# ypear/crdt

Measured on AMD Instinct MI355X. Metric: CRDT items merged/sec at 1/2/4/8 MI355X + % of HBM roofline, higher is better.
Workload: dtype u8/u32 (integer byte-stream + index work)

## Files before the change

crdt_amd/csrc/yc_decode.hip:

```cpp
#include <algorithm>
#include <cstdlib>

#include "yc_work.h"

namespace yc {

__device__ __forceinline__ uint64_t win8(const uint8_t* __restrict__ b, uint32_t p) {
  const uint32_t* d = (const uint32_t*)(b + (p & ~3u));
  return ((uint64_t)d[0] | ((uint64_t)d[1] << 32)) >> ((p & 3u) * 8);
}
__device__ __forceinline__ uint32_t win4(const uint8_t* __restrict__ b, uint32_t p) {
  const uint32_t* d = (const uint32_t*)(b + (p & ~3u));
  return __builtin_amdgcn_alignbyte(d[1], d[0], p & 3u);
}
struct RegWin {
  uint32_t r0, r1, r2, r3, r4, r5;
  uint32_t T;
  __device__ __forceinline__ static uint32_t sel(uint32_t m, uint32_t a1, uint32_t a0) { return (a1 & m) | (a0 & ~m); }
  __device__ __forceinline__ uint32_t word(uint32_t k) const {
    const uint32_t m0 = 0u - (k & 1u), m1 = 0u - ((k >> 1) & 1u), m2 = 0u - ((k >> 2) & 1u);
    const uint32_t a0 = sel(m0, r1, r0), a1 = sel(m0, r3, r2), a2 = sel(m0, r5, r4);
    return sel(m2, a2, sel(m1, a1, a0));
  }
  __device__ __forceinline__ uint32_t byte(uint32_t i) const { return (word(i >> 2) >> ((i & 3u) * 8)) & 0xFFu; }
// ... 3025 lines not shown
  const int pr = parse_struct<true, 32, WinSrc, DEFER>(WinSrc{bw, slot, s0}, p, uend, 0xFFFFFFFFu, &v);
  if (DEFER && pr == PARSE_DEFER) {
    w.sd_defer[atomicAdd(&w.ctr->nsd_defer, 1u)] = i;
    return;
  }
  if (pr <= 0) { raise_err(err, pr == -1 ? ERR_UNSUPPORTED : ERR_DECODE); return; }
  const uint32_t ref0 = v.ref;
  if (sec.pad && !w.lazy) {
    v.info = (uint8_t)((v.info & 0xE0u) | REF_SKIP);
    v.ref = REF_SKIP;
  }
  w.s_len[i] = v.len;
  w.s_info[i] = v.info;
  w.s_cidx[i] = sec.cidx;
  uint32_t oc = NONE, rc = NONE;
  const bool item = v.ref != REF_GC && v.ref != REF_SKIP;
  if (item && (v.info & 0x80u)) {
    oc = w.lazy ? v.oc : v.oc == sec.client ? sec.cidx : find_client(w, nclients, doc, v.oc);
    if (oc == NONE && !w.lazy) oc = UNKNOWN;
  }
  if (item && (v.info & 0x40u)) {
    rc = w.lazy ? v.rc : v.rc == sec.client ? sec.cidx : find_client(w, nclients, doc, v.rc);
    if (rc == NONE && !w.lazy) rc = UNKNOWN;
  }
  w.s_ocidx[i] = oc;
  w.s_oclock[i] = v.ok_;
  w.s_rcidx[i] = rc;
  if (rc != NONE) w.s_rclock[i] = v.rk;
  uint32_t pk = item ? v.pkind : 0u, pa = NONE, pb = 0;
  if (pk == 1) { pa = v.pa; pb = v.pb; }
  else if (pk == 2) {
    pa = w.lazy ? v.pa : v.pa == sec.client ? sec.cidx : find_client(w, nclients, doc, v.pa);
    pb = v.pb;
    if (pa == NONE && !w.lazy) pa = UNKNOWN;
  }
  if (pk != 0 && !v.has_psub) w.ctr->narray_roots = 1;
  if (pk == 2) w.ctr->nested = 1;
  wave_flag(&w.ctr->any_rorigin, item && (v.info & 0x40u));
  wave_count_add_sharded(w.ctr->nroots_sh, pk != 0);
  bool canon_hdr = true;
  if (item) {
    uint32_t h = 0;
    if (v.info & 0x80u) h += vu_size(v.oc) + vu_size(v.ok_);
    if (v.info & 0x40u) h += vu_size(v.rc) + vu_size(v.rk);
    if ((v.info & 0xC0u) == 0) {
      h += 1;
      if (v.pkind == 1) h += vu_size(v.pn) + v.pn;
      else h += vu_size(v.pa) + vu_size(v.pb);
      if (v.has_psub) h += vu_size(v.psn) + v.psn;
    }
    canon_hdr = h == v.cpos - p0 - 1;
  }
  w.s_pk[i] = (uint8_t)(pk | (canon_hdr ? 0u : 0x80u) | ((v.anyf & ANY_REENCODE) ? 0x40u : 0u) | ((v.anyf & ANY_KEYS) ? 0x20u : 0u));
  if (pk != 0) {
    w.s_pa[i] = pa;
    w.s_pb[i] = pb;
    w.s_psub[i] = v.has_psub ? v.psub_pos : NONE;
    w.s_psublen[i] = v.psub_len;
  }
  w.s_cpos[i] = v.cpos;
  w.s_cend[i] = v.cend;
  uint32_t celem = v.cpos;
  if (v.ref == REF_ANY || v.ref == REF_JSON) celem += vu_size(v.nel);
  w.s_celem[i] = celem;
  wave_flag(&w.ctr->any_json, ref0 == REF_JSON || ref0 == REF_EMBED || ref0 == REF_FORMAT || (v.anyf & ANY_KEYS) != 0);
}
__global__ __launch_bounds__(256) __attribute__((amdgpu_waves_per_eu(8, 8))) void k_struct_decode(Work w, uint32_t nstructs) {
  __shared__ __attribute__((aligned(16))) uint32_t win[256 * SD_STRIDE];
  const uint32_t i = blockIdx.x * blockDim.x + threadIdx.x;
  if (i < nstructs) struct_decode_one<true>(w, i, win);
}
constexpr uint32_t SD_DEFER_GRID = 1024;
__global__ __launch_bounds__(256) void k_struct_decode_deferred(Work w) {
  __shared__ __attribute__((aligned(16))) uint32_t win[256 * SD_STRIDE];
  const uint32_t n = w.ctr->nsd_defer;
  for (uint32_t k = blockIdx.x * blockDim.x + threadIdx.x; k < n; k += gridDim.x * blockDim.x)
    struct_decode_one<false>(w, w.sd_defer[k], win);
}
__global__ __launch_bounds__(256) void k_json_structs(Work w, uint32_t nstructs) {
  const uint32_t i = blockIdx.x * blockDim.x + threadIdx.x;
  if (i >= nstructs) return;
  const uint8_t* __restrict__ bw = struct_bytes(w, i);
  const uint32_t ref = bw[w.s_pos[i]] & 31u;
  if (w.ntrusted && w.sections[w.s_sec[i]].upd < w.ntrusted) return;
  if (ref == REF_ANY && (w.s_pk[i] & 0x20u)) {
    if (w.jskip_any) return;
    if (!any_keys_exact(bw, w.s_cpos[i], w.s_cend[i])) return;
    const uint32_t k = atomicAdd(&w.ctr->njson, 1u);
    if (k < w.jcap) w.jlist[k] = i;
    return;
  }
  if (ref != REF_JSON && ref != REF_EMBED && ref != REF_FORMAT) return;
  const int jr = json_content(bw, w.s_cpos[i], w.s_cend[i], ref);
  if (jr > 0) raise_err(&w.ctr->err, ERR_DECODE);
  if (jr < 0) {
    const uint32_t k = atomicAdd(&w.ctr->njson, 1u);
    if (k < w.jcap) w.jlist[k] = i;
  }
}
void launch_json_structs(const Work& w, uint32_t nstructs, hipStream_t s) {
  if (nstructs) hipLaunchKernelGGL(k_json_structs, dim3(nstructs / 256 + 1), dim3(256), 0, s, w, nstructs);
}
__global__ __launch_bounds__(64) void k_json_canon(Work w, const uint32_t* __restrict__ list, uint32_t n, JItem* __restrict__ items,
                                                   uint32_t* __restrict__ arena, uint32_t acap, uint32_t lanes,
                                                   const unsigned long long* __restrict__ offs, uint8_t* __restrict__ out) {
  const uint32_t t = blockIdx.x * blockDim.x + threadIdx.x;
  if (t >= lanes) return;
  uint32_t* a = arena + (uint64_t)t * acap;
  for (uint32_t j = t; j < n; j += lanes) {
    const uint32_t i = list[j];
    const uint8_t* __restrict__ bw = struct_bytes(w, i);
    const uint32_t ref = bw[w.s_pos[i]] & 31u, cp = w.s_cpos[i], ce = w.s_cend[i];
    uint32_t len = 0;
    if (!out) {
      const uint32_t r = json_content_canon(bw, cp, ce, ref, nullptr, a, acap, len);
      const unsigned long long base = w.nwin > 1 ? ((unsigned long long)w.s_win[i] << w.win_shift) : 0ull;
      items[j] = JItem{base + cp, ce - cp, len, r, 0u};
    } else if (items[j].res == JSON_OK) {
      uint8_t* o = out + offs[j];
      json_content_canon(bw, cp, ce, ref, o, a, acap, len);
      uint32_t same = len == ce - cp;
      for (uint32_t k = 0; same && k < len; ++k) same = o[k] == bw[cp + k];
      items[j].pad = same ? 0u : 1u;
    }
  }
}
void launch_json_canon(const Work& w, const uint32_t* list, uint32_t n, JItem* items, uint32_t* arena, uint32_t acap,
                       uint32_t lanes, const unsigned long long* offs, uint8_t* out, hipStream_t s) {
  if (n) hipLaunchKernelGGL(k_json_canon, dim3((lanes + 63) / 64), dim3(64), 0, s, w, list, n, items, arena, acap, lanes, offs, out);
}

__device__ __forceinline__ void struct_clock_at(const Work& w, uint32_t i, uint32_t nstructs, uint32_t states) {
  const uint32_t si = w.s_sec[i];
  const Section sec = w.sections[si];
  const uint64_t off = w.s_lenscan[i] - w.s_lenscan[sec.first_idx];
  const uint64_t clock = (uint64_t)sec.clock + off;
  const uint32_t len = w.s_len[i];
  const uint64_t endc = clock + len;
  if (endc > 0xFFFFFFFFull) { raise_err(&w.ctr->err, ERR_DECODE); return; }
  w.s_clock[i] = (uint32_t)clock;
  if (!states) return;
  const uint32_t ref = w.s_info[i] & 31u;
  if (ref == REF_SKIP) {
    atomicAdd(&w.ctr->items, (unsigned long long)len);
    return;
  }
  const bool last = i + 1 == nstructs || w.s_sec[i + 1] != si || (w.s_info[i + 1] & 31u) == REF_SKIP;
  if (last) atomicMax(&w.cl_state[w.s_cidx[i]], (uint32_t)endc);
}
__global__ void k_struct_clock(Work w, uint32_t nstructs, uint32_t states) {
  const uint32_t i = blockIdx.x * blockDim.x + threadIdx.x;
  if (i < nstructs) struct_clock_at(w, i, nstructs, states);
}

void launch_struct_decode(const Work& w, uint32_t nstructs, hipStream_t s) {
  if (!nstructs) return;
  hipLaunchKernelGGL(k_struct_decode, dim3((nstructs + 255) / 256), dim3(256), 0, s, w, nstructs);
  hipLaunchKernelGGL(k_struct_decode_deferred, dim3(std::min<uint32_t>(nstructs / 256 + 1, SD_DEFER_GRID)), dim3(256), 0, s, w);
}
void launch_struct_lenscan(const Work& w, uint32_t nstructs, hipStream_t s) {
  if (nstructs) scan_u32_to_u64(w.tmp, w.tmp_bytes, w.s_len, w.s_lenscan, nstructs + 1, s);
}

__device__ __forceinline__ void apply_caps_at(const Work& w, uint32_t c) {
  const uint32_t v = w.cl_vals[c];
  const uint32_t i = lower_bound_u32(w.cap_client, w.ncaps, v);
  const uint32_t cap = (i < w.ncaps && w.cap_client[i] == v) ? w.cap_clock[i] : 0u;
  if (ld_fresh(&w.cl_state[c]) > cap) w.cl_state[c] = cap;
}
__global__ void k_apply_caps(Work w) {
  const uint32_t c = blockIdx.x * blockDim.x + threadIdx.x;
  if (c < w.ctr->nclients) apply_caps_at(w, c);
}
__global__ void k_state_totals(Work w, uint32_t nstructs) {
  w.ctr->units = w.cl_base[w.ctr->nclients];
  w.ctr->in_len = w.s_lenscan[nstructs];
}
void launch_struct_clocks(const Work& w, uint32_t nstructs, hipStream_t s) {
  if (nstructs) hipLaunchKernelGGL(k_struct_clock, dim3((nstructs + 255) / 256), dim3(256), 0, s, w, nstructs, 0u);
}
void launch_states(const Work& w, uint32_t nstructs, uint32_t nsections, hipStream_t s) {
  if (nstructs) hipLaunchKernelGGL(k_struct_clock, dim3((nstructs + 255) / 256), dim3(256), 0, s, w, nstructs, 1u);
  if (w.capped && nsections) hipLaunchKernelGGL(k_apply_caps, dim3(nsections / 256 + 1), dim3(256), 0, s, w);
  scan_u32_to_u64(w.tmp, w.tmp_bytes, w.cl_state, w.cl_base, nsections + 1, s);
  hipLaunchKernelGGL(k_state_totals, dim3(1), dim3(1), 0, s, w, nstructs);
}

constexpr uint32_t DT_LANES = 256, DT_SMALL = 4096;
__global__ __launch_bounds__(DT_LANES) void k_decode_tail_small(Work w, uint32_t nstructs, uint32_t nsections) {
  __shared__ __attribute__((aligned(16))) uint32_t win[DT_LANES * SD_STRIDE];
  __shared__ uint64_t part[DT_LANES];
  const uint32_t t = threadIdx.x;
  if (nstructs == NONE) {
    if (w.ctr->err) return;
    nstructs = w.ctr->nstructs;
    nsections = w.ctr->nsections;
    if (nstructs > DT_SMALL || nsections + 1 > DT_LANES * 16) { if (t == 0) raise_err(&w.ctr->err, ERR_CAPACITY); return; }
  }
  if (w.dbg_bounds && (nstructs > w.cap_structs || nsections + 1 > w.cap_clients + 1)) {
    if (t == 0) bounds_fail(w.ctr, BOUNDS_DECODE_TAIL);
    return;
  }
  for (uint32_t i = t; i <= nsections; i += DT_LANES) { w.cl_start[i] = 0; w.cl_state[i] = 0; }
  for (uint32_t i = t; i < nstructs; i += DT_LANES) struct_decode_one<false>(w, i, win);
  __syncthreads();
  block_scan_u32_u64<DT_LANES>(w.s_len, w.s_lenscan, nstructs + 1, part);
  for (uint32_t i = t; i < nstructs; i += DT_LANES) struct_clock_at(w, i, nstructs, 1u);
  __syncthreads();
  const uint32_t nclients = w.ctr->nclients;
  if (w.capped) {
    for (uint32_t c = t; c < nclients; c += DT_LANES) apply_caps_at(w, c);
    __syncthreads();
  }
  block_scan_u32_u64<DT_LANES, true>(w.cl_state, w.cl_base, nsections + 1, part);
  if (t == 0) {
    w.ctr->units = w.cl_base[nclients];
    w.ctr->in_len = w.s_lenscan[nstructs];
  }
}
void launch_decode_tail_small(const Work& w, uint32_t nstructs, uint32_t nsections, hipStream_t s) {
  hipLaunchKernelGGL(k_decode_tail_small, dim3(1), dim3(DT_LANES), 0, s, w, nstructs, nsections);
}
bool decode_tail_small(const Work& w, uint32_t nstructs, uint32_t nsections, hipStream_t s) {
  const bool off = env_off("YCRDT_DECODE_SMALL");
  if (off || !nstructs || nstructs > DT_SMALL || nsections + 1 > DT_LANES * 16) return false;
  hipLaunchKernelGGL(k_decode_tail_small, dim3(1), dim3(DT_LANES), 0, s, w, nstructs, nsections);
  return true;
}

}
```

crdt_amd/csrc/yc_engine.hip:

```cpp
#include <cstddef>
#include <cstdio>
#include <cstring>
#include <string>
#include <vector>
#include <unordered_map>
#include <unordered_set>
#include <algorithm>
#include <memory>
#include <functional>

#include "yc_work.h"
#include "yc_host.h"
#include "yc_ingest.h"
#include "yc_comm.h"
#include <thread>
#include <atomic>
#include "../../include/ycrdt.h"

using namespace yc;

namespace {

thread_local std::string g_err;

// ... 948 lines not shown
  if (chunks) {
    HIPCHK(hipEventRecord(e->side_fork, s));
    HIPCHK(hipStreamWaitEvent(e->side, e->side_fork, 0));
    launch_chunks(wd, e->side);
    HIPCHK(hipEventRecord(e->side_done, e->side));
  }
  launch_direct(wd, s);
  mark(e, "decode.chunk_wait");
  if (chunks) HIPCHK(hipStreamWaitEvent(s, e->side_done, 0));
  if (split) {
    mark(e, "decode.exchange");
    const char* fh = getenv("YCRDT_TEST_FAIL_BEFORE_EXCHANGE");
    if (fh && fh[0] == '1') return fail(YCRDT_E_DEVICE, "test hook: failure before the decode exchange");
    const int rc0 = split_decode_exchange(e, b, sh);
    if (rc0 == YCRDT_E_CAPACITY && !generous) return run_decode(e, b, lazy, D, true, sh);
    if (rc0) return rc0;
  }
  mark(e, "decode.bitmap");
  if (!count_ds_small(w, s)) {
    launch_struct_count(w, s);
    launch_ds_bound(w, s);
  }
  if (!w.nupd) HIPCHK(hipMemcpyAsync(&w.ctr->nstructs, w.wcnt + (w.nbytes + 63) / 64, sizeof(uint32_t), hipMemcpyDeviceToDevice, s));
  Counters c;
  const bool quick = !lazy && !split && !generous && !w.dbg && !w.udoc && w.nupd && b->nwin <= 1 && w.nbytes <= (64u << 10) && w.cap_sections <= 16000 &&
                     !env_off("YCRDT_DECODE_SMALL") && !env_off("YCRDT_DECODE_QUICK");
  if (b->pre_src >= 0 && b->pre_check) launch_predecoded(w, b->pre_u, b->pre, true, s);
  int rc = quick ? YCRDT_OK : check(e, c, "decode");
  if (quick) {
    c = Counters();
    c.nstructs = (uint32_t)w.nbytes + 1;
    c.nsections = w.cap_sections;
    c.ds_region = (uint32_t)w.nbytes + w.nupd + 1;
  }
  if (dbg_dec && w.dbg) {
    unsigned long long h[24];
    HIPCHK(hipMemcpy(h, w.dbg, sizeof(h), hipMemcpyDeviceToHost));
    fprintf(stderr, "[ycrdt decode] multi-section fast walk cycles: stage %llu walk %llu search %llu, walked structs %llu, sections vouched %llu\n",
            h[19], h[20], h[21], h[22], h[23]);
    fprintf(stderr, "[ycrdt decode] fastwalk: done %llu nsec %llu unsynced %llu | wave: done %llu unsettled %llu other %llu (chunk path: moved / jumped chunk entries) | k_spec exact parses %llu (%llu bytes) | multi-section left to k_walk, by reason 1-5: %llu %llu %llu %llu %llu (section %llu of %llu structs) | record mode: %llu sections evaluated by the walker, stopped at byte %llu of %llu\n",
            h[0], h[1], h[2], h[3], h[4], h[5], h[6], h[7], h[9], h[10], h[11], h[12], h[13], h[14], h[15], h[16], h[17], h[18]);
    HIPCHK(hipMemsetAsync(w.dbg, 0, 192, s));
  }
  if (rc == YCRDT_E_CAPACITY && !generous) return run_decode(e, b, lazy, D, true, sh);
  if (rc) return rc;
  const uint32_t nstructs = c.nstructs;
  const uint32_t nsections = c.nsections;
  w.cap_structs = nstructs + 64;
  w.cap_ds = c.ds_region + 64;
  w.cap_clients = nsections + 64;
  w.ds = lazy ? take<DsRange>(V, B_DS, w.cap_ds, ok) : nullptr;
  w.ds_tmp = take<DsRange>(V, B_DSTMP, w.cap_ds, ok);
  w.ds_len = nullptr;
  w.s_pos = take<uint32_t>(V, B_SPOS, w.cap_structs, ok);
  w.s_win = b->nwin > 1 ? take<uint8_t>(V, B_SWIN, w.cap_structs, ok) : nullptr;
  w.s_sec = take<uint32_t>(V, B_SSEC, w.cap_structs, ok);
  w.s_len = take<uint32_t>(V, B_SLEN, w.cap_structs + 1, ok);
  w.s_lenscan = take<uint64_t>(V, B_SLENSCAN, w.cap_structs + 1, ok);
  w.s_clock = take<uint32_t>(V, B_SCLOCK, w.cap_structs, ok);
  w.s_cidx = take<uint32_t>(V, B_SCIDX, w.cap_structs, ok);
  w.s_info = take<uint8_t>(V, B_SINFO, w.cap_structs, ok);
  w.s_ocidx = take<uint32_t>(V, B_SOC, w.cap_structs, ok);
  w.s_oclock = take<uint32_t>(V, B_SOK, w.cap_structs, ok);
  w.s_rcidx = take<uint32_t>(V, B_SRC, w.cap_structs, ok);
  w.s_rclock = take<uint32_t>(V, B_SRK, w.cap_structs, ok);
  w.s_pk = take<uint8_t>(V, B_SPK, w.cap_structs, ok);
  w.s_pa = take<uint32_t>(V, B_SPA, w.cap_structs, ok);
  w.s_pb = take<uint32_t>(V, B_SPB, w.cap_structs, ok);
  w.s_psub = take<uint32_t>(V, B_SPS, w.cap_structs, ok);
  w.s_psublen = take<uint32_t>(V, B_SPL, w.cap_structs, ok);
  w.s_cpos = take<uint32_t>(V, B_SCPOS, w.cap_structs, ok);
  w.s_cend = take<uint32_t>(V, B_SCEND, w.cap_structs, ok);
  w.s_celem = take<uint32_t>(V, B_SCELEM, w.cap_structs, ok);
  w.sd_defer = take<uint32_t>(V, B_SDDEFER, w.cap_structs, ok);
  w.cl_vals = take<uint32_t>(V, B_CLVALS, w.cap_clients + 1, ok);
  w.ch_key = nullptr;
  const uint32_t ch_slots = (uint32_t)next_pow2(std::max<uint64_t>(2ull * (nsections + 1), 64));
  uint64_t* ch_key = take<uint64_t>(V, B_CHKEY, ch_slots, ok);
  uint32_t* ch_val = take<uint32_t>(V, B_CHVAL, ch_slots, ok);
  w.cl_key = take<uint64_t>(V, B_CLKEY, w.cap_clients + 1, ok);
  w.cl_key2 = take<uint64_t>(V, B_CLKEY2, w.cap_clients + 1, ok);
  w.cl_doc = take<uint32_t>(V, B_CLDOC, w.cap_clients + 1, ok);
  w.cl_tmp = take<uint32_t>(V, B_CLTMP, w.cap_clients + 1, ok);
  w.cl_state = take<uint32_t>(V, B_CLSTATE, w.cap_clients + 1, ok);
  w.cl_single = lazy ? nullptr : take<uint8_t>(V, B_CLSINGLE, w.cap_clients + 16, ok);
  w.cl_base = take<uint64_t>(V, B_CLBASE, w.cap_clients + 2, ok);
  w.cl_start = take<uint32_t>(V, B_CLSTART, w.cap_clients + 1, ok);
  if (!ok) return fail(YCRDT_E_DEVICE, oom("struct table"));
  launch_struct_scatter(w, s);
  const bool sec_small = quick || (!w.udoc && nsections && nsections <= 2048 && ch_slots <= 8192 && !env_off("YCRDT_DECODE_SMALL"));
  if (!sec_small) launch_section_clients(w, nsections, s);
  mark(e, "decode.sections");
  {
    Work wd = w;
    bool okd = true;
    if (quick) {
      HIPCHK(hipEventRecord(e->side_fork, s));
      HIPCHK(hipStreamWaitEvent(e->side, e->side_fork, 0));
    }
    wd.scratch = take<uint32_t>(V, B_SCRATCH2, (uint64_t)w.nupd + 2, okd);
    wd.tmp = take<uint8_t>(V, B_TMP2, prim_tmp_bytes(std::max<uint64_t>((uint64_t)w.nupd + 2, (uint64_t)w.ngroups + 2), 0), okd);
    wd.tmp_bytes = V[B_TMP2].cap;
    if (w.nbig) {
      wd.dsp_cnt = take<uint32_t>(V, B_DSPCNT, (uint64_t)w.ngroups + 1, okd);
      wd.dsp_pre = take<uint32_t>(V, B_DSPPRE, (uint64_t)w.ngroups + 1, okd);
      wd.dsp_val = take<uint32_t>(V, B_DSPVAL, 2ull * w.cap_ds, okd);
      wd.dsp_blk = take<uint4>(V, B_DSPBLK, (uint64_t)w.nbig * DSP_MAXBLK, okd);
      wd.dsp_nb = take<uint32_t>(V, B_DSPNB, w.nbig, okd);
      wd.dsp_gb = take<uint32_t>(V, B_DSPGB, (uint64_t)w.nbig + 1, okd);
      wd.dsp_b = take<uint32_t>(V, B_DSPB, (uint64_t)w.nupd + 1, okd);
      wd.dsp_fail = take<uint32_t>(V, B_DSPFAIL, (uint64_t)w.nupd + 1, okd);
      wd.dsp_j = take<uint32_t>(V, B_DSHJ, 2ull * w.cap_ds + 2, okd);
      wd.dsp_js = take<uint32_t>(V, B_DSHS, 2ull * w.cap_ds + 2, okd);
      wd.dsp_h = take<uint2>(V, B_DSHH, (uint64_t)w.nbig * (DSH_SEG + 1), okd);
      {
        uint64_t mx = 0;
        for (uint32_t i = 0; i < b->nbig; ++i) mx = std::max<uint64_t>(mx, b->ulen[b->ulist[i]]);
        wd.dsh_grid = (uint32_t)std::min<uint64_t>(256, mx / 512 + 1);
      }
      if (okd) fill_u32_multi({{wd.dsp_b, (uint64_t)w.nupd + 1, NONE}, {wd.dsp_fail, (uint64_t)w.nupd + 1, 0u}}, e->side);
    } else {
      wd.dsp_cnt = wd.dsp_pre = wd.dsp_val = wd.dsp_nb = wd.dsp_b = wd.dsp_fail = nullptr;
      wd.dsp_blk = nullptr;
      wd.dsp_j = wd.dsp_js = nullptr;
      wd.dsp_h = nullptr;
    }
    if (!okd) return fail(YCRDT_E_DEVICE, oom("delete-set scratch"));
    w.dsp_b = wd.dsp_b;
    launch_ds_decode(wd, e->side);
    HIPCHK(hipEventRecord(e->side_done, e->side));
  }
  if (sec_small) {
    if (!sections_small(w, quick ? NONE : nsections, ch_key, ch_val, ch_slots - 1, s)) return fail(YCRDT_E_DEVICE, "small section pass refused");
    w.ch_key = ch_key;
    w.ch_val = ch_val;
    w.ch_mask = ch_slots - 1;
  } else if (nsections) {
    launch_client_table(w, nsections, s);
    fill_u32_multi({{(uint32_t*)ch_key, 2ull * ch_slots, 0xFFFFFFFFu}}, s);
    launch_client_hash(w, ch_key, ch_val, ch_slots - 1, s);
    w.ch_key = ch_key;
    w.ch_val = ch_val;
    w.ch_mask = ch_slots - 1;
  }
  mark(e, "decode.structs");
  if (quick) {
    launch_decode_tail_small(w, NONE, NONE, s);
    mark(e, "decode.clocks");
  } else if (!lazy && decode_tail_small(w, nstructs, nsections, s)) {
    mark(e, "decode.clocks");
  } else {
  launch_struct_decode(w, nstructs, s);
  mark(e, "decode.clocks");
  launch_struct_lenscan(w, nstructs, s);
  if (!lazy) {
    fill_u32_multi({{w.cl_start, (uint64_t)nsections + 1, 0u}, {w.cl_state, (uint64_t)nsections + 1, 0u}}, s);
    launch_states(w, nstructs, nsections, s);
  } else {
    HIPCHK(hipMemsetAsync(w.cl_start, 0, sizeof(uint32_t) * (nsections + 1), s));
    launch_struct_clocks(w, nstructs, s);
  }
  }
  HIPCHK(hipStreamWaitEvent(s, e->side_done, 0));
  rc = check(e, c, "struct decode");
  if (quick && rc == YCRDT_E_CAPACITY) return run_decode(e, b, lazy, D, true, sh);
  if (rc) return rc;
  const uint32_t nstructs_q = quick ? c.nstructs : nstructs, nsections_q = quick ? c.nsections : nsections;
  if (c.any_json) {
    w.jcap = std::max<uint32_t>(nstructs_q, 1);
    w.jlist = take<uint32_t>(V, B_JLIST, w.jcap, ok);
    if (!ok) return fail(YCRDT_E_DEVICE, oom("JSON list"));
    w.ntrusted = b->ntrusted;
    w.jskip_any = b->jpasses > 0 ? 1u : 0u;
    launch_json_structs(w, nstructs_q, s);
    rc = check(e, c, "JSON values");
    if (rc) return rc;
    if (c.njson) {
      bool restaged = false;
      if ((rc = json_rewrite(e, b, std::min(c.njson, w.jcap), sh, restaged))) return rc;
      if (restaged) return run_decode(e, b, lazy, D, generous, sh);
    }
  }
  D.noncanon = c.noncanon;
  const uint32_t nclients = c.nclients;
  const uint64_t nunits = lazy ? 0 : c.units;
  D.in_len = c.in_len;
  D.array_roots = c.narray_roots;
  D.any_rorigin = c.any_rorigin;
  D.ds_big = c.ds_big != 0;
  D.nested = c.nested;
  D.nroots = 0;
  for (uint32_t k = 0; k < NSHARD; ++k) D.nroots += c.nroots_sh[k];
  if (nunits >= 0xF0000000ull) return fail(YCRDT_E_CAPACITY, "more than 2^32 units in one batch");
  D.nstructs = nstructs_q;
  D.nsections = nsections_q;
  D.nclients = nclients;
  D.nds = lazy ? std::min(c.nds, w.cap_ds) : c.ds_region;
  D.nunits = nunits;
  return YCRDT_OK;
}

int comm_allreduce_sum_u32(ycrdt_comm* c, uint32_t* buf, size_t n, hipStream_t s) {
  std::string err;
  if (yc::comm_allreduce_u32(c, buf, n, false, s, err)) return fail(YCRDT_E_DEVICE, err);
  return YCRDT_OK;
}
int run_merge(ycrdt_engine* e, ycrdt_batch* b, const std::unordered_map<uint32_t, uint32_t>* target,
              const ClockMap* caps = nullptr, const std::vector<uint32_t>* order = nullptr, const ShardSpec* sh = nullptr) {
  Work& w = e->w;
  auto& V = e->bufs;
  g_bufs = &V;
  bool ok = true;
  hipStream_t s = e->stream;
  e->ws_owner = nullptr;
  b->packed = false;
  w.capped = 0;
  w.ncaps = 0;
  if (caps) {
    uint32_t* cb = take<uint32_t>(V, B_CAPS, 2 * caps->size() + 2, ok);
    if (!ok) return fail(YCRDT_E_DEVICE, oom("caps"));
    std::vector<uint32_t> h(2 * caps->size() + 2, 0);
    size_t i = 0;
    for (const auto& kv : *caps) { h[i] = kv.first; h[caps->size() + i] = kv.second; ++i; }
    HIPCHK(hipMemcpyAsync(cb, h.data(), sizeof(uint32_t) * h.size(), hipMemcpyHostToDevice, s));
    w.cap_client = cb;
    w.cap_clock = cb + caps->size();
    w.ncaps = (uint32_t)caps->size();
    w.capped = 1;
  }
  Decoded D;
  int rc = run_decode(e, b, false, D, false, sh);
  if (rc) return rc;
  Counters c;
  const uint32_t nstructs = D.nstructs, nclients = D.nclients, nds = D.nds;
  const uint64_t nunits = D.nunits;
  const uint64_t B = (uint64_t)b->nbytes + 64;
  const uint64_t nwords = B / 64 + 2;
  std::vector<uint32_t> vals;
  if (((target && !target->empty()) || order) && nclients) {
    vals.resize(nclients);
    HIPCHK(hipMemcpy(vals.data(), w.cl_vals, sizeof(uint32_t) * nclients, hipMemcpyDeviceToHost));
  }
  w.cl_emit = w.cl_slot = nullptr;
  if (order && nclients) {
    std::unordered_map<uint32_t, uint32_t> rank;
    for (size_t i = 0; i < order->size(); ++i) rank.emplace((*order)[i], (uint32_t)i);
    std::vector<uint32_t> h(2 * (size_t)nclients);
    for (uint32_t c = 0; c < nclients; ++c) h[c] = c;
    std::stable_sort(h.begin(), h.begin() + nclients, [&](uint32_t a, uint32_t b2) {
      const auto ia = rank.find(vals[a]), ib = rank.find(vals[b2]);
      const uint32_t ra = ia == rank.end() ? UINT32_MAX : ia->second, rb = ib == rank.end() ? UINT32_MAX : ib->second;
      return ra < rb;
    });
    for (uint32_t i = 0; i < nclients; ++i) h[nclients + h[i]] = i;
    uint32_t* eb = take<uint32_t>(V, B_EMIT, h.size(), ok);
    if (!ok) return fail(YCRDT_E_DEVICE, oom("client order"));
    HIPCHK(hipMemcpyAsync(eb, h.data(), sizeof(uint32_t) * h.size(), hipMemcpyHostToDevice, s));
    w.cl_emit = eb;
    w.cl_slot = eb + nclients;
  }
  w.delta = target && !target->empty() && nclients ? 1u : 0u;
  if (target && !target->empty() && nclients) {
    std::vector<uint32_t> starts(nclients, 0);
    for (uint32_t i = 0; i < nclients; ++i) {
      auto it = target->find(vals[i]);
      if (it != target->end()) starts[i] = it->second;
    }
    HIPCHK(hipMemcpyAsync(w.cl_start, starts.data(), sizeof(uint32_t) * nclients, hipMemcpyHostToDevice, s));
  }
  const uint64_t U = nunits;
  const uint64_t uw = U / 64 + 2;
  w.cap_units = U + 1;
  w.u_owner = take<uint32_t>(V, B_UOWN, U + 1, ok);
  w.u_flags = take<uint32_t>(V, B_UFLAG, U + 1, ok);
  w.u_cutbits = take<uint64_t>(V, B_UCUT, uw, ok);
  w.u_wpre = take<uint32_t>(V, B_UWPRE, uw + 1, ok);
  w.scratch = take<uint32_t>(V, B_SCRATCH, std::max<uint64_t>({nwords + 2, (uint64_t)w.cap_sections + 66, uw + 2, U + 2}), ok);
  w.g_start = take<uint32_t>(V, B_GSTART, U + 2, ok);
  w.g_cidx = take<uint32_t>(V, B_GCIDX, U + 1, ok);
  w.g_src = take<uint32_t>(V, B_GSRC, U + 1, ok);
  w.g_flags = take<uint32_t>(V, B_GFLAGS, U + 1, ok);
  w.g_origin = take<uint32_t>(V, B_GORIG, U + 1, ok);
  w.g_rorigin = take<uint32_t>(V, B_GRORIG, U + 1, ok);
  w.g_hop = take<uint4>(V, B_GLINK, U + 1, ok);
  w.g_key = take<uint32_t>(V, B_GKEY, U + 1, ok);
  w.g_maxchild = take<uint32_t>(V, B_GMAXC, U + 1, ok);
  w.g_outid = take<uint32_t>(V, B_GOUTID, U + 2, ok);
  w.g_tmp = take<uint32_t>(V, B_GTMP, U + 2, ok);
  w.g_tmp2 = take<uint32_t>(V, B_GTMP2, U + 2, ok);
  w.o_first = take<uint32_t>(V, B_OFIRST, U + 2, ok);
  w.o_cidx = take<uint32_t>(V, B_OCIDX, U + 2, ok);
  w.o_size = take<uint32_t>(V, B_OSIZE, U + 2, ok);
  w.o_pos = take<uint32_t>(V, B_OPOS, U + 2, ok);
  w.o_gen = take<uint8_t>(V, B_OGEN, U + 32, ok);
  w.r_seg = take<uint32_t>(V, B_RSEG, U + 2, ok);
  w.r_len = take<uint32_t>(V, B_RLEN, U + 2, ok);
  w.r_size = take<uint32_t>(V, B_RSIZE, U + 2, ok);
  w.r_pos = take<uint32_t>(V, B_RPOS, U + 2, ok);
  w.cc = take<uint32_t>(V, B_CC, (size_t)CC_N * (w.cap_clients + 1), ok);
  w.cc64 = take<uint64_t>(V, B_CC64, (size_t)CC64_N * (w.cap_clients + 1), ok);
  {
    size_t tb = prim_tmp_bytes(std::max<uint64_t>({B / 64 + 4, U + 2, (uint64_t)nstructs + 2, 1024}), (uint64_t)D.nsections + 2);
    w.tmp = take<uint8_t>(V, B_TMP, tb, ok);
    w.tmp_bytes = V[B_TMP].cap;
  }
  if (!ok) return fail(YCRDT_E_DEVICE, oom("unit workspace"));
  mark(e, "merge.units_fill");
  if (U || nds) launch_units_fill(w, U, s);
  mark(e, "merge.units");
  {
    bool okt = true;
// ... 1941 lines not shown
```

crdt_amd/csrc/yc_work.h:

```cpp
#pragma once
#include <initializer_list>
#include "yc_common.h"
#include "yc_view.h"

namespace yc {

struct Counters {
  uint32_t err;
  uint32_t err_info;
  uint32_t nsections;
  uint32_t xchunks;
  uint32_t nds;
  uint32_t ndsclients;
  uint32_t nstructs;
  uint32_t nclients;
  uint32_t nunits_lo;
  uint32_t nunits_hi;
  uint32_t nsegs;
  uint32_t nout;
  uint32_t changed;
  uint32_t out_bytes;
  uint32_t sv_bytes;
  uint32_t nkeys;
  uint32_t nruns;
// ... 189 lines not shown
  uint32_t* y_iota = nullptr;
  uint32_t* y_lstart = nullptr;
  uint32_t* y_state = nullptr;
  uint32_t* y_before = nullptr;
  uint32_t* y_confl = nullptr;
  uint32_t* y_stack = nullptr;
  uint32_t* t_key = nullptr;
  uint32_t* t_keys = nullptr;
  uint32_t* t_seg = nullptr;
  uint32_t* t_pos = nullptr;
  uint32_t* t_gstart = nullptr;
  uint32_t* t_next = nullptr;
  uint32_t* t_done = nullptr;
  uint32_t* t_first = nullptr;
  uint32_t* t_nsib = nullptr;
  uint32_t* t_jump = nullptr;
  uint32_t* t_big = nullptr;
  uint32_t* t_prv = nullptr;
  uint32_t* t_mprv = nullptr;
  uint32_t* t_mtail = nullptr;
  uint32_t* t_otail = nullptr;
  uint32_t* t_hkey = nullptr;
  uint32_t* t_hval = nullptr;
  uint32_t* t_flag = nullptr;
  uint32_t* t_trep = nullptr;
  uint32_t* usec_start = nullptr;
  uint32_t* usec_n = nullptr;
  uint64_t* lz_key = nullptr;
  uint64_t* lz_keys = nullptr;
  uint32_t* lz_iota = nullptr;
  uint32_t* lz_sec = nullptr;
  uint32_t* lz_rstart = nullptr;
  uint32_t* lz_prev = nullptr;
  uint32_t* lz_first = nullptr;
  uint32_t* lz_cap = nullptr;
  uint32_t* lz_evbase = nullptr;
  uint32_t* lz_evn = nullptr;
  uint32_t* lz_flag = nullptr;
  uint32_t* lz_leave_hi = nullptr;
  uint32_t* lz_leave_lo = nullptr;
  uint32_t lz_nblk = 0, lz_diff = 0;
  uint32_t lz_multi = 0;
  uint32_t* lz_bclient = nullptr;
  uint32_t* ev_kind = nullptr;
  uint32_t* ev_src = nullptr;
  uint32_t* ev_clock = nullptr;
  uint32_t* ev_len = nullptr;
  uint32_t* ev_size = nullptr;
  uint32_t* ev_pos = nullptr;
  uint32_t* blk_size = nullptr;
  uint32_t* blk_pos = nullptr;
  const uint32_t* sv_client = nullptr;
  const uint32_t* sv_clock = nullptr;
  uint32_t sv_n = 0;
  const uint32_t* sv_off = nullptr;
  uint64_t* dsm_key = nullptr;
  uint64_t* dsm_keys = nullptr;
  uint32_t* dsm_len = nullptr;
  uint32_t* dsm_lens = nullptr;
  uint64_t* dsm_end = nullptr;
  uint64_t* dsm_max = nullptr;
  uint32_t* dsm_flag = nullptr;
  uint32_t* dsm_rid = nullptr;
  uint32_t* dr_client = nullptr;
  uint32_t* dr_clock = nullptr;
  uint32_t* dr_end = nullptr;
  uint32_t* dw_flag = nullptr;
  uint32_t* dw_gid = nullptr;
  uint32_t* dw_gstart = nullptr;
  uint32_t* dw_size = nullptr;
  uint32_t* dw_pos = nullptr;
  uint32_t ds_first = 0;
  uint32_t* ds_fa = nullptr;
  uint32_t* o_first = nullptr;
  uint32_t* o_cidx = nullptr;
  uint32_t* o_size = nullptr;
  uint32_t* o_pos = nullptr;
  uint8_t* o_gen = nullptr;
  uint32_t* r_seg = nullptr;
  uint32_t* r_len = nullptr;
  uint32_t* r_size = nullptr;
  uint32_t* r_pos = nullptr;
  uint32_t* cc = nullptr;
  uint64_t* cc64 = nullptr;
  const uint32_t* cl_emit = nullptr;
  const uint32_t* cl_slot = nullptr;
  uint32_t cap_clients = 0;
  uint8_t* out = nullptr;
  uint64_t cap_out = 0;
  uint64_t cap_sv = 0;
  uint8_t* sv_out = nullptr;
  uint32_t* scratch = nullptr;
  void* tmp = nullptr;
  size_t tmp_bytes = 0;
};

__device__ __forceinline__ uint32_t xcd_block() {
  const uint32_t b = blockIdx.x, G = gridDim.x, per = G >> 3, rem = G & 7u, x = b & 7u;
  return x * per + min(x, rem) + (b >> 3);
}
__device__ __forceinline__ uint32_t gidx() { return xcd_block() * blockDim.x + threadIdx.x; }

struct OrderedIds {
  unsigned long long* ctr = nullptr;
  unsigned long long base = 0;
};
bool ordered_ids(uint64_t nblocks, hipStream_t s, OrderedIds& out);
__device__ __forceinline__ uint32_t ordered_block_id(unsigned long long* ctr, unsigned long long base) {
  __shared__ uint32_t id;
  if (threadIdx.x == 0) id = (uint32_t)(atomicAdd(ctr, 1ull) - base);
  __syncthreads();
  return id;
}

constexpr uint64_t LB_VAL = (1ull << 40) - 1;
struct LbChains {
  unsigned long long* state = nullptr;
  uint64_t stride = 0;
  uint32_t epoch = 0;
  unsigned long long* ord = nullptr;
  unsigned long long ord_base = 0;
};
bool lb_launch(uint64_t tiles, uint32_t chains, hipStream_t s, LbChains& out);
__device__ __forceinline__ uint64_t lb_wave_lookback(unsigned long long* __restrict__ state, uint32_t tile, uint32_t epoch, uint64_t agg) {
  const uint32_t lane = threadIdx.x & 63;
  const unsigned long long ep = (unsigned long long)epoch << 42;
  if (tile == 0) {
    if (lane == 0) __hip_atomic_store(&state[0], ep | (2ull << 40) | (agg & LB_VAL), __ATOMIC_RELAXED, __HIP_MEMORY_SCOPE_AGENT);
    return 0;
  }
  if (lane == 0) __hip_atomic_store(&state[tile], ep | (1ull << 40) | (agg & LB_VAL), __ATOMIC_RELAXED, __HIP_MEMORY_SCOPE_AGENT);
  uint64_t pre = 0;
  for (int64_t j = (int64_t)tile - 1;; j -= 64) {
    const int64_t me = j - (int64_t)lane;
    uint32_t st = 2;
    uint64_t val = 0;
    if (me >= 0) {
      unsigned long long x;
      while (((x = __hip_atomic_load(&state[me], __ATOMIC_RELAXED, __HIP_MEMORY_SCOPE_AGENT)) >> 42) != epoch)
        __builtin_amdgcn_s_sleep(1);
      st = (uint32_t)(x >> 40) & 3u;
      val = x & LB_VAL;
    }
    const uint64_t done = __ballot(st == 2);
    const uint32_t stop = (uint32_t)__ffsll((long long)done) - 1;
    uint64_t part = lane <= stop ? val : 0ull;
    for (uint32_t off = 32; off > 0; off >>= 1) part += __shfl_xor(part, off);
    pre += part;
    if (done) break;
  }
  if (lane == 0) __hip_atomic_store(&state[tile], ep | (2ull << 40) | ((pre + agg) & LB_VAL), __ATOMIC_RELAXED, __HIP_MEMORY_SCOPE_AGENT);
  return pre;
}

__device__ __forceinline__ uint64_t client_hash(uint64_t k) {
  k ^= k >> 30; k *= 0xBF58476D1CE4E5B9ull;
  k ^= k >> 27; k *= 0x94D049BB133111EBull;
  return k ^ (k >> 31);
}
__device__ __forceinline__ uint32_t find_client(const Work& w, uint32_t nclients, uint32_t doc, uint32_t client) {
  if (w.ch_key) {
    const uint64_t key = w.udoc ? (((uint64_t)doc << 32) | client) : (uint64_t)client;
    for (uint32_t slot = (uint32_t)client_hash(key) & w.ch_mask;; slot = (slot + 1) & w.ch_mask) {
      const uint64_t k = w.ch_key[slot];
      if (k == key) return w.ch_val[slot];
      if (k == ~0ull) return NONE;
    }
  }
  if (!w.udoc) {
    const uint32_t i = lower_bound_u32(w.cl_vals, nclients, client);
    return (i < nclients && w.cl_vals[i] == client) ? i : NONE;
  }
  const uint64_t key = ((uint64_t)doc << 32) | client;
  uint32_t lo = 0, hi = nclients;
  while (lo < hi) { const uint32_t m = (lo + hi) >> 1; if (w.cl_key[m] < key) lo = m + 1; else hi = m; }
  return (lo < nclients && w.cl_key[lo] == key) ? lo : NONE;
}
__device__ __forceinline__ uint32_t doc_of_update(const Work& w, uint32_t upd) { return w.udoc ? w.udoc[upd] : 0u; }
__device__ __forceinline__ uint32_t seg_start(const Work& w, uint32_t s) { return w.g_start[s]; }
__device__ __forceinline__ uint32_t seg_of_unit(const Work& w, uint32_t g) {
  return w.u_wpre[g >> 6] + (uint32_t)__popcll(w.u_cutbits[g >> 6] & ((2ull << (g & 63)) - 1)) - 1;
}
__device__ __forceinline__ uint32_t upd_win(const Work& w, uint32_t upd) { return w.uwin ? w.uwin[upd] : 0u; }
__device__ __forceinline__ const uint8_t* win_bytes(const Work& w, uint32_t win) { return w.bytes + ((uint64_t)win << w.win_shift); }
#define win_words(bits, win) ((bits) + ((uint64_t)(win) << (w.win_shift - 6)))
__device__ __forceinline__ const uint8_t* struct_bytes(const Work& w, uint32_t s) {
  return w.nwin > 1 ? win_bytes(w, w.s_win[s]) : w.bytes;
}

static __device__ __attribute__((noinline)) uint64_t content_slice_walk(const uint8_t* __restrict__ by, uint32_t ref, uint32_t celem,
                                                                        uint32_t cpos, uint32_t end, uint32_t e0, uint32_t e1);
__device__ __forceinline__ bool content_slice(const Work& w, uint32_t src, uint32_t e0, uint32_t e1, uint32_t& b0, uint32_t& b1) {
  const uint32_t ref = w.s_info[src] & 31u;
  if (e0 == 0 && e1 == w.s_len[src] && (ref == REF_ANY || ref == REF_JSON)) {
    b0 = w.s_celem[src];
    b1 = w.s_cend[src];
    return true;
  }
  const uint64_t r = content_slice_walk(struct_bytes(w, src), ref, w.s_celem[src], w.s_cpos[src], w.s_cend[src], e0, e1);
  if (r == ~0ull) return false;
  b0 = (uint32_t)r;
  b1 = (uint32_t)(r >> 32);
  return true;
}
static __device__ __attribute__((noinline)) uint64_t content_slice_walk(const uint8_t* __restrict__ by, uint32_t ref, uint32_t celem,
                                                                        uint32_t cpos, uint32_t end, uint32_t e0, uint32_t e1) {
  uint32_t b0 = 0, b1 = 0;
  const bool got = [&]() -> bool {
  if (ref == REF_ANY || ref == REF_JSON) {
    uint32_t p = celem;
    bool ok = true;
    for (uint32_t i = 0; i < e1; ++i) {
      if (i == e0) b0 = p;
      if (ref == REF_ANY) {
        uint32_t steps = 0xFFFFFFFFu;
        ok = skip_any<32>(by, p, end, steps);
      } else {
        const uint32_t k = rd_vu(by, p, end, ok);
        if (ok) skip_bytes(p, k, end, ok);
      }
      if (!ok) return false;
    }
    if (e0 == e1) b0 = p;
    b1 = p;
    return true;
  }
  if (ref == REF_STRING) {
    uint32_t p = cpos;
    bool ok = true;
    rd_vu(by, p, end, ok);
    if (!ok) return false;
    uint32_t u = 0;
    b0 = e0 == 0 ? p : NONE;
    while (p < end && u < e1) {
      const uint32_t c = by[p];
      const uint32_t n = c < 0x80u ? 1u : c < 0xE0u ? 2u : c < 0xF0u ? 3u : 4u;
      const uint32_t du = n == 4 ? 2u : 1u;
      if (u < e0 && u + du > e0) return false;
      if (u < e1 && u + du > e1) return false;
      p += n;
      u += du;
      if (u == e0) b0 = p;
    }
    b1 = p;
    return b0 != NONE && u == e1;
  }
  b0 = cpos;
  b1 = end;
  return true;
  }();
  return got ? ((uint64_t)b1 << 32) | b0 : ~0ull;
}

template <bool WRITE>
__device__ __attribute__((noinline)) uint32_t any_canon(const uint8_t* __restrict__ by, uint32_t p, uint32_t end, uint32_t e0,
                                                        uint32_t e1, uint8_t* __restrict__ out, uint64_t q0) {
  uint64_t q = q0;
  auto put = [&](uint32_t x) { if (WRITE) out[q] = (uint8_t)x; ++q; };
  auto put_vu = [&](uint32_t v) { while (v > 0x7Fu) { put(0x80u | (v & 0x7Fu)); v >>= 7; } put(v); };
  auto put_vi = [&](bool neg, uint32_t m) {
    put((m > 63u ? 0x80u : 0u) | (neg ? 0x40u : 0u) | (m & 63u));
    m >>= 6;
    while (m) { put((m > 127u ? 0x80u : 0u) | (m & 127u)); m >>= 7; }
  };
  auto put_num = [&](double x) {
    const uint32_t k = num_form(x);
    if (k == 0) { put(125); put_vi(x < 0 || (x == 0 && signbit(x)), (uint32_t)fabs(x)); return; }
    if (k == 1) { union { float f; uint32_t u; } c; c.f = (float)x; put(124); for (int s = 24; s >= 0; s -= 8) put((c.u >> s) & 0xFFu); return; }
    union { double d; uint64_t u; } c; c.d = x;
    put(123);
    for (int s = 56; s >= 0; s -= 8) put((uint32_t)(c.u >> s) & 0xFFu);
  };
  bool ok = true;
  uint32_t rem[33];
  uint32_t objm = 0;
  int d = 0;
  rem[0] = e1;
  uint32_t idx = 0;
  for (;;) {
    if (d == 0 && idx >= e1) break;
    const bool emit = idx >= e0;
    const uint32_t tag = by[p++];
    const uint32_t s0 = p;
    switch (tag) {
      case 127: case 126: case 121: case 120: if (emit) put(tag); break;
      case 125: {
        skip_vi(by, p, end, ok);
        bool neg;
        const uint32_t m = vi_decode(by, s0, p, neg);
        if (emit) { if (!neg && m > 0x7FFFFFFFu) put_num((double)m); else { put(125); put_vi(neg, m); } }
        break;
      }
      case 124: p += 4; if (emit) put_num(f32_of(be32(by, s0))); break;
      case 123: p += 8; if (emit) put_num(f64_of(be64(by, s0))); break;
      case 122: p += 8; if (emit) { put(122); for (uint32_t i = s0; i < p; ++i) put(by[i]); } break;
      case 119: case 116: {
        const uint32_t n = rd_vu(by, p, end, ok);
        if (emit) { put(tag); put_vu(n); for (uint32_t i = 0; i < n; ++i) put(by[p + i]); }
        p += n;
        break;
      }
      default: {
        const uint32_t n = rd_vu(by, p, end, ok);
        if (emit) { put(tag); put_vu(n); }
        if (n > 0) {
          if (d >= 32) return 0;
// ... 190 lines not shown
```

Before: 3.867 billion.

## Fuse struct length scan and clock assignment into one decoupled-lookback segmented scan

Result: no change. 3.915 billion, median of 6 (+1.2%).

```diff
diff --git a/crdt_amd/csrc/yc_decode.hip b/crdt_amd/csrc/yc_decode.hip
--- a/crdt_amd/csrc/yc_decode.hip
+++ b/crdt_amd/csrc/yc_decode.hip
@@ -3201,6 +3201,119 @@
   const uint32_t i = blockIdx.x * blockDim.x + threadIdx.x;
   if (i < nstructs) struct_clock_at(w, i, nstructs, states);
 }
+constexpr uint32_t SC_ITEMS = 16, SC_TILE = 256 * SC_ITEMS;
+constexpr uint64_t SC_SAT = 1ull << 33;
+__device__ __forceinline__ uint64_t sc_add(uint64_t a, uint64_t b) { return a + b < SC_SAT ? a + b : SC_SAT; }
+__global__ __launch_bounds__(256) void k_clock_scan(Work w, uint32_t nstructs, uint32_t vec, LbChains lb) {
+  __shared__ uint64_t wval[4], wlen[4];
+  __shared__ uint32_t whead[4];
+  __shared__ uint64_t tile_in;
+  const uint32_t tile = ordered_block_id(lb.ord, lb.ord_base);
+  const uint32_t t = threadIdx.x, lane = t & 63, wv = t >> 6;
+  const uint64_t base = (uint64_t)tile * SC_TILE + (uint64_t)t * SC_ITEMS;
+  const bool full = base + SC_ITEMS <= nstructs;
+  uint32_t len[SC_ITEMS], sec[SC_ITEMS], iw[SC_ITEMS / 4];
+  if (vec && full) {
+    const uint4 iq = *(const uint4*)(w.s_info + base);
+    iw[0] = iq.x; iw[1] = iq.y; iw[2] = iq.z; iw[3] = iq.w;
+#pragma unroll
+    for (uint32_t k = 0; k < SC_ITEMS / 4; ++k) {
+      const uint4 a = ((const uint4*)(w.s_len + base))[k], b = ((const uint4*)(w.s_sec + base))[k];
+      len[4 * k] = a.x; len[4 * k + 1] = a.y; len[4 * k + 2] = a.z; len[4 * k + 3] = a.w;
+      sec[4 * k] = b.x; sec[4 * k + 1] = b.y; sec[4 * k + 2] = b.z; sec[4 * k + 3] = b.w;
+    }
+  } else {
+#pragma unroll
+    for (uint32_t k = 0; k < SC_ITEMS / 4; ++k) iw[k] = 0;
+#pragma unroll
+    for (uint32_t k = 0; k < SC_ITEMS; ++k) {
+      const bool in = base + k < nstructs;
+      len[k] = in ? w.s_len[base + k] : 0u;
+      sec[k] = in ? w.s_sec[base + k] : NONE;
+      iw[k >> 2] |= (in ? (uint32_t)w.s_info[base + k] : 0u) << (8 * (k & 3u));
+    }
+  }
+  const uint32_t psec = base > 0 && base - 1 < nstructs ? w.s_sec[base - 1] : NONE;
+  const bool more = base + SC_ITEMS < nstructs;
+  const uint32_t nsec = more ? w.s_sec[base + SC_ITEMS] : NONE;
+  const uint32_t ninfo = more ? w.s_info[base + SC_ITEMS] & 31u : 0u;
+  uint32_t heads = 0;
+#pragma unroll
+  for (uint32_t k = 0; k < SC_ITEMS; ++k)
+    if (base + k < nstructs && sec[k] != (k ? sec[k - 1] : psec)) heads |= 1u << k;
+  if (base == 0 && nstructs) heads |= 1u;
+  uint64_t v = 0, tot = 0;
+#pragma unroll
+  for (uint32_t k = 0; k < SC_ITEMS; ++k) {
+    if ((heads >> k) & 1u) v = w.sections[sec[k]].clock;
+    v = sc_add(v, len[k]);
+    tot += len[k];
+  }
+  bool h = heads != 0;
+  const uint64_t own = v;
+  const bool ownh = h;
+  for (uint32_t off = 1; off < 64; off <<= 1) {
+    const uint64_t yv = __shfl_up(v, off);
+    const uint32_t yh = __shfl_up(h ? 1u : 0u, off);
+    if (lane >= off) {
+      if (!h) v = sc_add(yv, v);
+      h = h || yh;
+    }
+  }
+  for (uint32_t off = 32; off > 0; off >>= 1) tot += __shfl_xor(tot, off);
+  if (lane == 63) { wval[wv] = v; whead[wv] = h ? 1u : 0u; }
+  if (lane == 0) wlen[wv] = tot;
+  uint64_t ev = __shfl_up(v, 1u);
+  uint32_t eh = __shfl_up(h ? 1u : 0u, 1u);
+  if (lane == 0) { ev = 0; eh = 0; }
+  __syncthreads();
+  uint64_t pv = 0, tv = 0;
+  uint32_t ph = 0, th = 0;
+#pragma unroll
+  for (uint32_t k = 0; k < 4; ++k) {
+    if (k == wv) { pv = tv; ph = th; }
+    tv = whead[k] ? wval[k] : sc_add(tv, wval[k]);
+    th |= whead[k];
+  }
+  if (!eh) { ev = sc_add(pv, ev); eh = ph; }
+  if (wv == 0) {
+    const uint64_t pre = lb_wave_lookback_seg(lb.state, tile, lb.epoch, tv, th != 0, SC_SAT);
+    if (lane == 0) {
+      tile_in = pre;
+      atomicAdd(&w.ctr->in_len, (unsigned long long)(wlen[0] + wlen[1] + wlen[2] + wlen[3]));
+    }
+  }
+  __syncthreads();
+  uint64_t run = eh ? ev : sc_add(tile_in, ev);
+  uint32_t o[SC_ITEMS];
+#pragma unroll
+  for (uint32_t k = 0; k < SC_ITEMS; ++k) {
+    if ((heads >> k) & 1u) run = w.sections[sec[k]].clock;
+    const uint64_t endc = run + len[k];
+    o[k] = (uint32_t)run;
+    if (base + k < nstructs) {
+      if (endc > 0xFFFFFFFFull) {
+        raise_err(&w.ctr->err, ERR_DECODE);
+      } else if (((iw[k >> 2] >> (8 * (k & 3u))) & 31u) == REF_SKIP) {
+        atomicAdd(&w.ctr->items, (unsigned long long)len[k]);
+      } else {
+        const bool nh = k + 1 < SC_ITEMS ? ((heads >> ((k + 1) & 15u)) & 1u) != 0 : nsec != sec[k];
+        const uint32_t ni = k + 1 < SC_ITEMS ? (iw[((k + 1) & 15u) >> 2] >> (8 * ((k + 1) & 3u))) & 31u : ninfo;
+        if (base + k + 1 == nstructs || nh || ni == REF_SKIP) atomicMax(&w.cl_state[w.sections[sec[k]].cidx], (uint32_t)endc);
+      }
+    }
+    run = sc_add(run, len[k]);
+  }
+  if (vec && full) {
+#pragma unroll
+    for (uint32_t k = 0; k < SC_ITEMS / 4; ++k)
+      ((uint4*)(w.s_clock + base))[k] = make_uint4(o[4 * k], o[4 * k + 1], o[4 * k + 2], o[4 * k + 3]);
+  } else {
+#pragma unroll
+    for (uint32_t k = 0; k < SC_ITEMS; ++k)
+      if (base + k < nstructs) w.s_clock[base + k] = o[k];
+  }
+}
 
 void launch_struct_decode(const Work& w, uint32_t nstructs, hipStream_t s) {
   if (!nstructs) return;
@@ -3221,18 +3334,31 @@
   const uint32_t c = blockIdx.x * blockDim.x + threadIdx.x;
   if (c < w.ctr->nclients) apply_caps_at(w, c);
 }
-__global__ void k_state_totals(Work w, uint32_t nstructs) {
+__global__ void k_state_totals(Work w, uint32_t nstructs, uint32_t lenscan) {
   w.ctr->units = w.cl_base[w.ctr->nclients];
-  w.ctr->in_len = w.s_lenscan[nstructs];
+  if (lenscan) w.ctr->in_len = w.s_lenscan[nstructs];
 }
 void launch_struct_clocks(const Work& w, uint32_t nstructs, hipStream_t s) {
   if (nstructs) hipLaunchKernelGGL(k_struct_clock, dim3((nstructs + 255) / 256), dim3(256), 0, s, w, nstructs, 0u);
 }
 void launch_states(const Work& w, uint32_t nstructs, uint32_t nsections, hipStream_t s) {
-  if (nstructs) hipLaunchKernelGGL(k_struct_clock, dim3((nstructs + 255) / 256), dim3(256), 0, s, w, nstructs, 1u);
+  bool scanned = false;
+  if (nstructs && !env_off("YCRDT_CLOCK_SCAN")) {
+    const uint32_t tiles = (nstructs + SC_TILE - 1) / SC_TILE;
+    const uint32_t vec = (((uintptr_t)w.s_len | (uintptr_t)w.s_sec | (uintptr_t)w.s_info | (uintptr_t)w.s_clock) & 15u) == 0;
+    LbChains lb;
+    if (lb_launch(tiles, 1, s, lb)) {
+      hipLaunchKernelGGL(k_clock_scan, dim3(tiles), dim3(256), 0, s, w, nstructs, vec, lb);
+      scanned = true;
+    }
+  }
+  if (nstructs && !scanned) {
+    launch_struct_lenscan(w, nstructs, s);
+    hipLaunchKernelGGL(k_struct_clock, dim3((nstructs + 255) / 256), dim3(256), 0, s, w, nstructs, 1u);
+  }
   if (w.capped && nsections) hipLaunchKernelGGL(k_apply_caps, dim3(nsections / 256 + 1), dim3(256), 0, s, w);
   scan_u32_to_u64(w.tmp, w.tmp_bytes, w.cl_state, w.cl_base, nsections + 1, s);
-  hipLaunchKernelGGL(k_state_totals, dim3(1), dim3(1), 0, s, w, nstructs);
+  hipLaunchKernelGGL(k_state_totals, dim3(1), dim3(1), 0, s, w, nstructs, scanned ? 0u : 1u);
 }
 
 constexpr uint32_t DT_LANES = 256, DT_SMALL = 4096;
diff --git a/crdt_amd/csrc/yc_engine.hip b/crdt_amd/csrc/yc_engine.hip
--- a/crdt_amd/csrc/yc_engine.hip
+++ b/crdt_amd/csrc/yc_engine.hip
@@ -1124,11 +1124,11 @@
   } else {
   launch_struct_decode(w, nstructs, s);
   mark(e, "decode.clocks");
-  launch_struct_lenscan(w, nstructs, s);
   if (!lazy) {
     fill_u32_multi({{w.cl_start, (uint64_t)nsections + 1, 0u}, {w.cl_state, (uint64_t)nsections + 1, 0u}}, s);
     launch_states(w, nstructs, nsections, s);
   } else {
+    launch_struct_lenscan(w, nstructs, s);
     HIPCHK(hipMemsetAsync(w.cl_start, 0, sizeof(uint32_t) * (nsections + 1), s));
     launch_struct_clocks(w, nstructs, s);
   }
diff --git a/crdt_amd/csrc/yc_work.h b/crdt_amd/csrc/yc_work.h
--- a/crdt_amd/csrc/yc_work.h
+++ b/crdt_amd/csrc/yc_work.h
@@ -365,6 +365,40 @@
   if (lane == 0) __hip_atomic_store(&state[tile], ep | (2ull << 40) | ((pre + agg) & LB_VAL), __ATOMIC_RELAXED, __HIP_MEMORY_SCOPE_AGENT);
   return pre;
 }
+__device__ __forceinline__ uint64_t lb_wave_lookback_seg(unsigned long long* __restrict__ state, uint32_t tile, uint32_t epoch, uint64_t agg,
+                                                         bool head, uint64_t sat) {
+  const uint32_t lane = threadIdx.x & 63;
+  const unsigned long long ep = (unsigned long long)epoch << 42;
+  if (tile == 0) {
+    if (lane == 0) __hip_atomic_store(&state[0], ep | (2ull << 40) | agg, __ATOMIC_RELAXED, __HIP_MEMORY_SCOPE_AGENT);
+    return 0;
+  }
+  if (lane == 0) __hip_atomic_store(&state[tile], ep | ((head ? 2ull : 1ull) << 40) | agg, __ATOMIC_RELAXED, __HIP_MEMORY_SCOPE_AGENT);
+  uint64_t pre = 0;
+  for (int64_t j = (int64_t)tile - 1;; j -= 64) {
+    const int64_t me = j - (int64_t)lane;
+    uint32_t st = 2;
+    uint64_t val = 0;
+    if (me >= 0) {
+      unsigned long long x;
+      while (((x = __hip_atomic_load(&state[me], __ATOMIC_RELAXED, __HIP_MEMORY_SCOPE_AGENT)) >> 42) != epoch)
+        __builtin_amdgcn_s_sleep(1);
+      st = (uint32_t)(x >> 40) & 3u;
+      val = x & LB_VAL;
+    }
+    const uint64_t done = __ballot(st == 2);
+    const uint32_t stop = (uint32_t)__ffsll((long long)done) - 1;
+    uint64_t part = lane <= stop ? val : 0ull;
+    for (uint32_t off = 32; off > 0; off >>= 1) part += __shfl_xor(part, off);
+    pre = pre + part < sat ? pre + part : sat;
+    if (done) break;
+  }
+  if (!head && lane == 0) {
+    const uint64_t inc = pre + agg < sat ? pre + agg : sat;
+    __hip_atomic_store(&state[tile], ep | (2ull << 40) | inc, __ATOMIC_RELAXED, __HIP_MEMORY_SCOPE_AGENT);
+  }
+  return pre;
+}
 
 __device__ __forceinline__ uint64_t client_hash(uint64_t k) {
   k ^= k >> 30; k *= 0xBF58476D1CE4E5B9ull;
```
